# pmelchior/scarlet

Hardware: AMD Instinct MI355X
Metric: PGM iters/sec over batched blends; achieved HBM GB/s vs roofline (higher is better)
Workload: dtype f32; 1 GPU; configs[2]: 1024 independent 5-band 128x128 blends in total, 10 ExtendedSource components (41x41) each, ConvolutionRenderer FFT 160x160; iterations 0..1234 of a fit from the initial parameters; loop=blend, blends_total=1024, components_per_blend=10, sub_ranges_per_gpu=3

## Files before the change

include/scarlet_amd.h:

```cpp
#ifndef SCARLET_AMD_H
#define SCARLET_AMD_H

#include <stdint.h>

#ifdef __cplusplus
extern "C" {
#endif

typedef enum smi_status {
    SMI_OK = 0,
    SMI_ERR_INVALID = -1,
    SMI_ERR_HIP = -2,
    SMI_ERR_NO_DEVICE = -3,
    SMI_ERR_ARITHMETIC = -4
} smi_status;

const char *smi_last_error(void);
int smi_device_count(void);
const char *smi_version(void);


int smi_prox_weighted_monotonic_f32(float *flat_img, const float *weights,
                                    const int32_t *offsets, int32_t n_off,
                                    const int32_t *dist_idx, int32_t n_idx,
// ... 382 lines not shown
int smi_batch_set_iteration_base(smi_batch *b, const int32_t *base);
int smi_batch_get_progress(smi_batch *b, int32_t *state, int32_t *n_loss);
int smi_batch_set_pause_at(smi_batch *b, const int32_t *it);
int smi_batch_get_converged(smi_batch *b, int32_t *flag);
int smi_batch_set_round(smi_batch *b, const int32_t *state, const int32_t *base,
                        const int32_t *pause_at);
int smi_batch_get_round(smi_batch *b, int32_t *state, int32_t *n_loss, int32_t *converged);

int64_t smi_observation_uploads(void);

int smi_batch_conv_path_used(smi_batch *b, int32_t *path);

int smi_batch_set_frame_extents(smi_batch *b, const int32_t *h, const int32_t *w);

int smi_fft_shape_for(int32_t H, int32_t W, int32_t kernel_h, int32_t kernel_w, int32_t conv_path,
                      int32_t *Fy, int32_t *Fx);

typedef struct smi_resampler smi_resampler;
int smi_resampler_create(const float *A, const float *Pt, int32_t C, int32_t n_a, int32_t n_b,
                         int32_t Fy, int32_t Fx, smi_resampler **out);
int smi_resampler_render(smi_resampler *r, const float *model, float *out);
int smi_resampler_time(smi_resampler *r, int32_t n_rep, double *ms_per_render);
int smi_resampler_destroy(smi_resampler *r);
int smi_resampler_get_path(smi_resampler *r, int32_t *path);
int smi_resampler_set_path(smi_resampler *r, int32_t path);

int smi_gemm_plan(int32_t M, int32_t N, int32_t K, int32_t n_batch, int64_t scratch_elems,
                  int32_t plan[5]);
int smi_gemm_test(const float *A, int64_t strideA, const float *B, int64_t strideB, float *C,
                  int64_t strideC, int32_t n_batch, int32_t M, int32_t N, int32_t K,
                  int64_t scratch_elems, int32_t plan[5], int32_t *guard_ok);
int smi_resampler_adjoint(smi_resampler *r, const float *resid, float *gpad);

int smi_batch_attach_lowres(smi_batch *b, smi_resampler *r, const int32_t *channels,
                            const float *data, const float *weights, double log_norm);
int smi_batch_get_lowres_rendered(smi_batch *b, int32_t index, float *out);


int smi_starlet_transform_f32(const float *d_images, int32_t n, int32_t H, int32_t W,
                              int32_t scales, int32_t generation, double *d_coeffs,
                              double *d_work, void *stream);
int smi_starlet_transform_f64(const double *d_images, int32_t n, int32_t H, int32_t W,
                              int32_t scales, int32_t generation, double *d_coeffs,
                              double *d_work, void *stream);
int smi_starlet_reconstruction_f64(const double *d_coeffs, int32_t n, int32_t H, int32_t W,
                                   int32_t scales, int32_t generation, double *d_image,
                                   double *d_work, void *stream);
int smi_multiresolution_support_f64(const double *d_coeffs, int32_t n, int32_t planes,
                                    int32_t H, int32_t W, int64_t plane_stride,
                                    int64_t image_stride, const double *sigma0,
                                    const double *thresh0, double K, double epsilon,
                                    int32_t max_iter, int32_t *d_support, double *d_masked,
                                    int32_t *iterations, void *stream);
int smi_coadd_f32(const float *d_images, int32_t bands, int32_t H, int32_t W, float *d_out,
                  void *stream);
int smi_coadd_f64(const double *d_images, int32_t bands, int32_t H, int32_t W, double *d_out,
                  void *stream);

typedef struct smi_detect_task {
    int32_t bands, h, w, scales;
    int64_t image_off, coeff_off, work_off;
    double sigma0, thresh0;
} smi_detect_task;
int smi_detect_wavelets_scratch_bytes(int32_t n, int64_t *bytes);
int smi_detect_wavelets_f32(int32_t n, const smi_detect_task *tasks, const void *d_tasks, double K,
                            double epsilon, int32_t max_iter, int32_t generation,
// ... 71 lines not shown
```

scarlet_amd/_lib.py:

```python

import ctypes
import os

import numpy as np

_HERE = os.path.dirname(os.path.abspath(__file__))
LIB_PATH = os.environ.get("SCARLET_AMD_LIB") or os.path.join(_HERE, "libscarlet_amd.so")

PROX_MONOTONIC = 1
PROX_SYMMETRY = 2
PROX_POSITIVE = 4
PROX_CENTER_ON = 8
PROX_NORM_MAX = 16
PROX_NORM_SUM = 32
PROX_L1 = 64
PROX_L0 = 128
PROX_FIT_CENTER = 256
PROX_BG_THRESH = 512
PROX_L_RELATIVE = 1024
PROX_MONO_MASK = 2048
SCHEME_AMSGRAD, SCHEME_FISTA = 0, 1
COMPONENT_POINT_SOURCE = 1 << 16
COMPONENT_SHIFTING = 1 << 17
COMPONENT_FIXED_SED = 1 << 18
# ... 129 lines not shown
    "smi_get_valid_monotonic_pixels_f64": (
        ctypes.c_int,
        [ctypes.c_int32, ctypes.c_int32, c_f64p, ctypes.c_int32, ctypes.c_int32, c_u8p, c_u8p,
         ctypes.c_double, c_i32p, ctypes.c_double],
    ),
    "smi_linear_interpolate_invalid_pixels_f32": (
        ctypes.c_int,
        [c_i32p, c_i32p, ctypes.c_int32, c_u8p, c_f32p, ctypes.c_int32, ctypes.c_int32, c_u8p,
         ctypes.c_double, ctypes.c_int32, c_i32p],
    ),
    "smi_linear_interpolate_invalid_pixels_f64": (
        ctypes.c_int,
        [c_i32p, c_i32p, ctypes.c_int32, c_u8p, c_f64p, ctypes.c_int32, ctypes.c_int32, c_u8p,
         ctypes.c_double, ctypes.c_int32, c_i32p],
    ),
    "smi_resampler_create": (
        ctypes.c_int,
        [c_f32p, c_f32p, ctypes.c_int32, ctypes.c_int32, ctypes.c_int32, ctypes.c_int32,
         ctypes.c_int32, ctypes.POINTER(ctypes.c_void_p)],
    ),
    "smi_resampler_render": (ctypes.c_int, [ctypes.c_void_p, c_f32p, c_f32p]),
    "smi_resampler_time": (ctypes.c_int, [ctypes.c_void_p, ctypes.c_int32,
                                          ctypes.POINTER(ctypes.c_double)]),
    "smi_resampler_destroy": (ctypes.c_int, [ctypes.c_void_p]),
    "smi_resampler_get_path": (ctypes.c_int, [ctypes.c_void_p, ctypes.POINTER(ctypes.c_int32)]),
    "smi_resampler_set_path": (ctypes.c_int, [ctypes.c_void_p, ctypes.c_int32]),
    "smi_resampler_adjoint": (ctypes.c_int, [ctypes.c_void_p, c_f32p, c_f32p]),
    "smi_gemm_plan": (ctypes.c_int, [ctypes.c_int32] * 4 + [ctypes.c_int64, c_i32p]),
    "smi_gemm_test": (
        ctypes.c_int,
        [c_f32p, ctypes.c_int64, c_f32p, ctypes.c_int64, c_f32p, ctypes.c_int64]
        + [ctypes.c_int32] * 4 + [ctypes.c_int64, c_i32p, c_i32p],
    ),
    "smi_batch_attach_lowres": (
        ctypes.c_int, [ctypes.c_void_p, ctypes.c_void_p, c_i32p, c_f32p, c_f32p, ctypes.c_double]
    ),
    "smi_batch_get_lowres_rendered": (ctypes.c_int, [ctypes.c_void_p, ctypes.c_int32, c_f32p]),
    "smi_batch_create": (
        ctypes.c_int,
        [ctypes.POINTER(BatchDesc), ctypes.c_int, ctypes.POINTER(ctypes.c_void_p)],
    ),
    "smi_batch_destroy": (ctypes.c_int, [ctypes.c_void_p]),
    "smi_batch_add_sweep_plan": (
        ctypes.c_int,
        [ctypes.c_void_p, ctypes.c_int32, ctypes.c_int32, c_f64p, c_i32p, c_i32p,
         ctypes.c_int32],
    ),
    "smi_sweep_ring_plan": (
        ctypes.c_int,
        [ctypes.c_int32, ctypes.c_int32, c_f64p, c_i32p, c_i32p, ctypes.c_int32, c_i32p, c_f32p,
         ctypes.POINTER(ctypes.c_uint16), ctypes.c_int64],
    ),
    "smi_batch_set_observation": (ctypes.c_int, [ctypes.c_void_p, c_f32p, c_f32p]),
    "smi_batch_set_observation_device": (
        ctypes.c_int, [ctypes.c_void_p, ctypes.c_void_p, ctypes.c_void_p]
    ),
    "smi_batch_set_kernel": (ctypes.c_int, [ctypes.c_void_p, c_f32p]),
    "smi_batch_set_components": (ctypes.c_int, [ctypes.c_void_p, ctypes.POINTER(Components)]),
    "smi_batch_set_moments": (ctypes.c_int, [ctypes.c_void_p] + [c_f32p] * 6),
    "smi_batch_get_moments": (ctypes.c_int, [ctypes.c_void_p] + [c_f32p] * 6),
    "smi_batch_get_parameters": (ctypes.c_int, [ctypes.c_void_p, c_f32p, c_f32p]),
    "smi_batch_set_parameters": (ctypes.c_int, [ctypes.c_void_p, c_f32p, c_f32p]),
    "smi_batch_get_centers": (ctypes.c_int, [ctypes.c_void_p] + [c_f64p] * 5),
    "smi_batch_set_center_moments": (ctypes.c_int, [ctypes.c_void_p] + [c_f64p] * 3),
    "smi_batch_set_centers": (ctypes.c_int, [ctypes.c_void_p, c_f64p]),
    "smi_batch_get_model_morphology": (ctypes.c_int, [ctypes.c_void_p, c_f32p]),
# ... 235 lines not shown
```

scarlet_amd/csrc/batch.hip:

```cpp
#include <rocfft/rocfft.h>

#include <algorithm>
#include <cmath>
#include <cstdlib>
#include <atomic>
#include <cstring>
#include <limits>
#include <map>
#include <mutex>
#include <thread>
#include <tuple>
#include <utility>

#include "common.h"

namespace smi {

static thread_local std::string g_error;
static std::atomic<int> g_hw_queues{4};
static std::atomic<long long> g_observation_uploads{0};
static std::mutex g_plan_mutex;
void set_error(const std::string &msg) { g_error = msg; }

static int next_fast_len(int n) {
// ... 597 lines not shown
}

int smi_resampler_adjoint(smi_resampler *r, const float *resid, float *gpad) {
    SMI_REQUIRE(r && r->impl && resid && gpad, "null argument");
    return resampler_adjoint_host(r->impl, resid, gpad);
}

int smi_gemm_plan(int32_t M, int32_t N, int32_t K, int32_t n_batch, int64_t scratch_elems,
                  int32_t plan[5]) {
    SMI_REQUIRE(plan && scratch_elems >= 0, "bad argument");
    GemmPlan p;
    const int rc = gemm_plan(M, N, K, n_batch, (size_t)scratch_elems, &p);
    plan[0] = p.tm; plan[1] = p.tn; plan[2] = p.bk; plan[3] = p.kslice; plan[4] = p.n_slices;
    return rc;
}

int smi_gemm_test(const float *A, int64_t strideA, const float *B, int64_t strideB, float *C,
                  int64_t strideC, int32_t n_batch, int32_t M, int32_t N, int32_t K,
                  int64_t scratch_elems, int32_t plan[5], int32_t *guard_ok) {
    SMI_REQUIRE(A && B && C && plan && guard_ok && scratch_elems >= 0, "bad argument");
    int ndev = 0;
    if (hipGetDeviceCount(&ndev) != hipSuccess || ndev == 0) {
        set_error("no HIP device available");
        return SMI_ERR_NO_DEVICE;
    }
    GemmPlan p;
    *guard_ok = 0;
    const int rc = gemm_test(A, strideA, B, strideB, C, strideC, n_batch, M, N, K,
                             (size_t)scratch_elems, &p, guard_ok);
    plan[0] = p.tm; plan[1] = p.tn; plan[2] = p.bk; plan[3] = p.kslice; plan[4] = p.n_slices;
    return rc;
}

static constexpr int kMaxLowRes = 8;

int smi_batch_attach_lowres(smi_batch *b, smi_resampler *r, const int32_t *channels,
                            const float *data, const float *weights, double log_norm) {
    SMI_REQUIRE(b && r && channels && data && weights, "null argument");
    SMI_REQUIRE(b->d.n_blends == 1, "a low-resolution observation needs a batch of one blend");
    SMI_REQUIRE(!b->frame_hw, "a low-resolution observation does not support frame extents");
    SMI_REQUIRE(r->impl, "resampler already destroyed");
    SMI_REQUIRE((int)b->lowres.size() < kMaxLowRes, "too many low-resolution observations");
    SMI_HIP(hipSetDevice(b->device));
    SMI_HIP(hipStreamSynchronize(b->stream));
    if (!b->extra_terms) {
        SMI_HIP(dev_alloc(&b->extra_terms, kMaxLowRes));
        SMI_HIP(hipMemset(b->extra_terms, 0, kMaxLowRes * sizeof(double)));
    }
    LowRes *l = nullptr;
    int rc = lowres_create(r->impl, channels, data, weights, log_norm, b->d.H, b->d.W,
                           b->extra_terms + b->lowres.size(), &l);
    if (rc) {
        lowres_destroy(l);
        return rc;
    }
    b->lowres.push_back(l);
    refresh_view(b);
    return SMI_OK;
}

int smi_batch_get_lowres_rendered(smi_batch *b, int32_t index, float *out) {
    SMI_REQUIRE(b && out, "null argument");
    SMI_REQUIRE(index >= 0 && index < (int)b->lowres.size(), "no such low-resolution observation");
    return lowres_get_rendered(b->lowres[index], out, b->stream);
}

// ... 2320 lines not shown
```

scarlet_amd/csrc/common.h:

```cpp
#pragma once

#include <hip/hip_runtime.h>
#include <stdint.h>

#include <string>
#include <vector>

#include "../../include/scarlet_amd.h"

namespace smi {

void set_error(const std::string &msg);

#define SMI_HIP(expr)                                                              \
    do {                                                                           \
        hipError_t _e = (expr);                                                    \
        if (_e != hipSuccess) {                                                    \
            smi::set_error(std::string(#expr) + ": " + hipGetErrorString(_e));     \
            return SMI_ERR_HIP;                                                    \
        }                                                                          \
    } while (0)

#define SMI_REQUIRE(cond, msg)                                                     \
    do {                                                                           \
// ... 265 lines not shown
                            uint8_t *unchecked, uint8_t *orphans, double variance,
                            int32_t *bounds, double thresh);
template <typename T>
int mask_interpolate_host_buffers(const int32_t *row_idx, const int32_t *col_idx, int32_t n_idx,
                                  uint8_t *unchecked, T *model, int32_t rows, int32_t cols,
                                  uint8_t *orphans, double variance, int32_t recursive,
                                  int32_t *bounds);
struct Resampler;
int resampler_create(const float *A, const float *Pt, int C, int n_a, int n_b, int Fy, int Fx,
                     Resampler **out);
int resampler_render(Resampler *r, const float *model, float *out);
int resampler_time(Resampler *r, int n_rep, double *ms_per_render);
int resampler_get_path(const Resampler *r);
int resampler_set_path(Resampler *r, int path);
void resampler_destroy(Resampler *r);
int resampler_adjoint_host(Resampler *r, const float *resid, float *gpad);
struct GemmPlan {
    int32_t tm = 0, tn = 0, bk = 0, kslice = 0, n_slices = 0;
};
int gemm_plan(int M, int N, int K, int n_batch, size_t scratch_elems, GemmPlan *p);
int gemm_test(const float *A, int64_t strideA, const float *B, int64_t strideB, float *C,
              int64_t strideC, int n_batch, int M, int N, int K, size_t scratch_elems,
              GemmPlan *plan, int32_t *guard_ok);
struct LowRes;
int lowres_create(Resampler *r, const int32_t *channels, const float *data, const float *weights,
                  double log_norm, int H, int W, double *term_slot, LowRes **out);
void lowres_destroy(LowRes *l);
int lowres_evaluate(LowRes *l, const float *P, int Py, int Px, int backward, hipStream_t s);
void lowres_add_gradient(LowRes *l, float *Q, int Py, int Px, hipStream_t s);
int lowres_get_rendered(LowRes *l, float *out, hipStream_t s);
int launch_sweep_timing(const SweepPlanDev *d_plans, const SweepPlanDev &host_plan, int plan_id,
                        int mode, int n_rep, float one_minus_g, int waves, int groups,
                        long long *cycles, float *images, hipStream_t s);
void launch_resize_test(const BatchView &v, int32_t *margin, double *pull, hipStream_t s);
void launch_gather_states(const BatchView &v, const int32_t *sel, const int64_t *off, int32_t n_sel,
                          float *staging, hipStream_t s);
void launch_scatter_states(const BatchView &v, const int64_t *off, const float *staging,
                           hipStream_t s);
void launch_carry_states(const int32_t *keep, const int64_t *old_moff, const int64_t *new_moff,
                         int32_t n, float *const from[4], float *const to[4], hipStream_t s);
void launch_interleave_obs(const float *data, const float *weights, float4 *dw, int64_t planes,
                           int32_t H, int32_t W, hipStream_t s);
void launch_log_norm(const float *weights, double *log_norm, int32_t nb, int64_t n,
                     hipStream_t s);
void launch_wrap_kernel(const float *kern, float *out, int32_t n_img, int32_t ph,
                        int32_t pw, int32_t Fy, int32_t Fx, float scale, hipStream_t s);
void launch_crop(const float *P, float *out, int32_t n_img, int32_t H, int32_t W,
                 int32_t Fy, int32_t Fx, hipStream_t s);
void launch_count_active(const int32_t *state, int32_t nb, int32_t *out, hipStream_t s);

bool fused_conv_supported(int Fy, int Fx);
bool fused_conv_instantiated(int Fy, int Fx);
bool fused_conv_choose(int ny, int nx, int *Fy, int *Fx);
int launch_fused_conv(const BatchView &v, int Fy, int Fx, const float *model, const float2 *Kt,
                      int k_bands, int k_per_blend, float *out, int mode, long long *dbg,
                      hipStream_t s);
int launch_fused_conv_short(const BatchView &v, int Fy, int Fx, const float *model,
                            const float2 *Kt, int k_bands, int k_per_blend, float *out, int mode,
                            long long *dbg, hipStream_t s);
int launch_stamp_spectrum(const float *d_kern, double2 *d_tmp, float2 *Kt, int n_img, int ph,
                          int pw, int Fy, int Fx, double scale, hipStream_t s);
int launch_permute_kernel_spectrum(const float2 *Khat, float2 *Kt, int n_img, int Fy, int Fx,
                                   float scale, hipStream_t s);

template <typename T>
int sweep_host_buffers(T *flat_img, int32_t n_pix, const SweepPlanHost &plan, T min_gradient);
// ... 10 lines not shown
```

scarlet_amd/csrc/kernels.hip:

```cpp
#include <math.h>

#include <algorithm>
#include <type_traits>
#include <stdlib.h>

#include "common.h"
#include "rounded_math.h"

namespace smi {

namespace {

constexpr int kBandChunk = 8;
constexpr int kPixBlock = 256;

template <int CTRL>
__device__ __forceinline__ float dpp_f(float v) {
    return __int_as_float(__builtin_amdgcn_update_dpp(0, __float_as_int(v), CTRL, 0xf, 0xf, false));
}
__device__ __forceinline__ float wave_sum(float v) {
    v += dpp_f<0xB1>(v);
    v += dpp_f<0x4E>(v);
    v += dpp_f<0x141>(v);
    v += dpp_f<0x140>(v);
// ... 1273 lines not shown
    const RingGlobal<1> plan(stream, bytes, n_pad, lane);
    if (kLate && n_nat < n_pad)
        sweep_ring_loop<1, true, RingGlobal<1>>(us, plan, n_pad, n_nat, rmax, perm, centre,
                                                one_minus_g, lane);
    else
        sweep_ring_loop<1, false, RingGlobal<1>>(us, plan, n_pad, n_pad, rmax, perm, centre,
                                                 one_minus_g, lane);
}

#ifndef SMI_XP_TEAM
#define SMI_XP_TEAM 1
#endif
constexpr bool update_xp(int team) { return SMI_XP_TEAM && team > 64; }
constexpr int update_waves(int npl, int team) {
    return npl <= 16 ? 4 : npl <= 27 ? (update_xp(team) ? 4 : 3) : 2;
}
#ifndef SMI_WAVES
#define SMI_WAVES __attribute__((amdgpu_waves_per_eu(update_waves(NPL, T))))
#endif
template <int NPL, bool XP>
struct UpdState {
    CompCtx c;
    int k, flags, plan_id, bad, ctr, n_slots;
    float xs[XP ? 1 : NPL], rs[XP ? 1 : NPL], zs[NPL];
    float rpmax;
    bool fista_prox;
    float alpha, pmax, t_old;
    bool monotonic, fit_center;
    bool std_chain;
    const SweepSlotEntry *slots;
    const SweepPlanDev *ring;
    const SweepPlanDev *staged;
    const char *plan_lds;
    float one_minus_g, lthresh, cfloor, pfloor;
    const float *bg_level;
    float *us, *sed_new;
};

constexpr bool update_lean(int npl, int mode, int team) {
    return mode != 2 && !(team == 256 && npl == 16);
}
template <int T, bool LEAN>
__device__ __forceinline__ uint32_t slot_offset(int lane, uint32_t lane4, int j) {
    return LEAN ? lane4 + (uint32_t)(T * j) * 4u : (uint32_t)(lane + T * j) * 4u;
}
template <int NPL>
struct UpdFull {
    static constexpr int value = NPL == 7 ? 0 : NPL == 16 ? 7 : NPL == 27 ? 16 : NPL == 42 ? 27 : 42;
};

template <int NPL, int MODE, int T, bool EXT>
__device__ __forceinline__ void upd_step(const BatchView &v, const float *G, int it, float e2,
                                         int prox_max_iter, UpdState<NPL, update_xp(T)> &S) {
    constexpr bool LITE = MODE != 0;
    constexpr bool fista = MODE == 2;
    constexpr bool XP = update_xp(T);
    constexpr int kFull = UpdFull<NPL>::value;
    constexpr bool LEAN = update_lean(NPL, MODE, T);
    const CompCtx &c = S.c;
    it = v.local_it(c.b, it);
    const int lane = c.lane, k = S.k, N = c.N;
    const uint32_t lane4 = lane_byte_offset(lane);
    float *us = S.us;
    float xs_local[NPL], rs_local[NPL];
    auto &xs = [&]() -> float(&)[NPL] {
        if constexpr (XP) return xs_local;
        else return S.xs;
    }();
    auto &rs = [&]() -> float(&)[NPL] {
        if constexpr (XP) return rs_local;
        else return S.rs;
    }();
    float(&zs)[NPL] = S.zs;
    const int flags = S.flags = v.c_flags[k];
    const int plan_id = S.plan_id = v.c_plan[k];
    const uint32_t nbytes = (uint32_t)N * 4u;

    {
        const rsrc_t r_morph = make_rsrc(c.morph, nbytes);
#pragma unroll
        for (int j = 0; j < NPL; ++j) zs[j] = buf_load(r_morph, slot_offset<T, LEAN>(lane, lane4, j));
    }
    float g_sed = 0.f;
    if (c.pre) {
        const rsrc_t r_g = make_rsrc(v.g_morph_buf + c.moff, nbytes);
#pragma unroll
        for (int j = 0; j < NPL; ++j) xs[j] = buf_load(r_g, slot_offset<T, LEAN>(lane, lane4, j));
        g_sed = lane < c.C ? v.g_sed_buf[(int64_t)k * c.C + lane] : 0.f;
    } else {
        uint32_t *goff = reinterpret_cast<uint32_t *>(us);
        const float inv_w = 1.0f / (float)c.w;
        const int Hb = EXT ? v.frame_h(c.b) : v.H, Wb = EXT ? v.frame_w(c.b) : v.W;
#pragma unroll
        for (int j = 0; j < NPL; ++j) {
            const int i = lane + T * j;
            const int y = (int)(((float)i + 0.5f) * inv_w);
            const int x = i - y * c.w;
            const int fy = y + c.oy, fx = x + c.ox;
            const bool ok = (j < kFull || i < N) && (unsigned)fy < (unsigned)Hb &&
                            (unsigned)fx < (unsigned)Wb;
            goff[i] = ok ? (uint32_t)(fy * v.Fx + fx) * 4u : kOutOfRange;
            xs[j] = 0.f;
        }
        const int64_t plane = (int64_t)v.Fy * v.Fx;
        for (int cb = 0; cb < c.C; ++cb) {
            const rsrc_t r_g = make_rsrc(G + ((int64_t)c.b * c.C + cb) * plane, (uint32_t)plane * 4u);
            float g[NPL];
#pragma unroll
            for (int j = 0; j < NPL; ++j) g[j] = buf_load(r_g, goff[lane + T * j]);
            const float s = c.sed[cb];
            float acc = 0.f;
#pragma unroll
            for (int j = 0; j < NPL; ++j) {
                xs[j] = fmaf(s, g[j], xs[j]);
                acc = fmaf(g[j], zs[j], acc);
            }
            const float t = Team<T>::sum(acc);
            if (lane == cb) g_sed = t;
        }
    }
    if (flags & SMI_COMPONENT_FIXED_MORPH) {
#pragma unroll
        for (int j = 0; j < NPL; ++j) xs[j] = 0.f;
    }
    if (flags & SMI_COMPONENT_FIXED_SED) g_sed = 0.f;

    float msum = 0.f, msum2 = 0.f;
#pragma unroll
    for (int j = 0; j < NPL; ++j) {
        msum += zs[j];
        msum2 = fmaf(zs[j], zs[j], msum2);
    }
    float ssum2 = 1.f;
    S.t_old = 1.f;
    if (fista) {
        msum2 = Team<T>::sum(msum2);
        const float so = lane < c.C ? c.sed[lane] : 0.f;
        ssum2 = Team<T>::sum(so * so);
        S.t_old = (float)v.fista_t[2 * (int64_t)k + 1];
    }
    S.bad = 0;
    if (T == 64 || threadIdx.x < 64)
        S.bad = update_spectrum(v, c, g_sed, it, e2, prox_max_iter, msum2, S.sed_new);
    const float alpha = fmaxf(v.c_morph_step[k], v.c_morph_rel[k] * (Team<T>::sum(msum) / (float)N));
    float pmax = 0.f;
    const rsrc_t r_m = make_rsrc(v.m_morph + c.moff, nbytes);
    const rsrc_t r_x = make_rsrc(v.xp_tmp + c.moff, nbytes);
    const rsrc_t r_p = make_rsrc(v.xp_tmp + v.n_morph_total + c.moff, nbytes);
    S.fista_prox = fista;
    if (fista) {
        const float step = v.c_fista_step[k] / ssum2;
        if constexpr (XP) {
#pragma unroll
            for (int j = 0; j < NPL; ++j) zs[j] = buf_load(r_m, slot_offset<T, LEAN>(lane, lane4, j));
#pragma unroll
            for (int j = 0; j < NPL; ++j) zs[j] = zs[j] - step * xs[j];
        } else {
#pragma unroll
            for (int j = 0; j < NPL; ++j) rs[j] = buf_load(r_m, slot_offset<T, LEAN>(lane, lane4, j));
#pragma unroll
            for (int j = 0; j < NPL; ++j) {
                xs[j] = rs[j] - step * xs[j];
                rs[j] = 0.f;
                zs[j] = xs[j];
            }
        }
        pmax = 1.f;
    } else {
        const rsrc_t r_v = make_rsrc(v.v_morph + c.moff, nbytes);
        const rsrc_t r_vh = make_rsrc(v.vh_morph + c.moff, nbytes);
        constexpr int CH = NPL <= 6 ? NPL : 6;
        const float b1 = v.b1, b2 = v.b2, eps = v.eps;
        float cm[CH], cv[CH], cvh[CH];
#pragma unroll
        for (int u = 0; u < CH; ++u) {
            const uint32_t off = slot_offset<T, LEAN>(lane, lane4, u);
            cm[u] = buf_load(r_m, off);
            cv[u] = buf_load(r_v, off);
            cvh[u] = buf_load(r_vh, off);
        }
#pragma unroll
        for (int j0 = 0; j0 < NPL; j0 += CH) {
            float nm[CH], nv[CH], nvh[CH];
#pragma unroll
            for (int u = 0; u < CH; ++u) {
                nm[u] = nv[u] = nvh[u] = 0.f;
                if (j0 + CH + u < NPL) {
                    const uint32_t off = slot_offset<T, LEAN>(lane, lane4, (j0 + CH + u));
                    nm[u] = buf_load(r_m, off);
                    nv[u] = buf_load(r_v, off);
                    nvh[u] = buf_load(r_vh, off);
                }
            }
#pragma unroll
            for (int u = 0; u < CH; ++u) {
                const int j = j0 + u;
                if (j < NPL) {
                    const uint32_t off = slot_offset<T, LEAN>(lane, lane4, j);
                    const float g = xs[j];
                    const float m = (1.f - b1) * g + b1 * cm[u];
                    const float vv = (1.f - b2) * g * g + b2 * cv[u];
                    const float vh = it == 0 ? vv : fmaxf(cvh[u], vv);
                    buf_store(r_m, off, m);
                    buf_store(r_v, off, vv);
                    buf_store(r_vh, off, vh);
                    const float psi = sqrtf(fmaxf(vh, eps));
                    float upd = alpha * m / psi;
                    if (it == 0) upd /= 10.f;
                    xs[j] = zs[j] - upd;
                    zs[j] = xs[j];
                    const bool in_box = j < kFull || lane + T * j < N;
                    if constexpr (XP) {
                        const float rj = in_box ? psi : 0.f;
                        buf_store(r_x, off, xs[j]);
                        buf_store(r_p, off, rj);
                        pmax = fmaxf(pmax, rj);
                    } else {
                        rs[j] = in_box ? psi : 0.f;
                        pmax = fmaxf(pmax, rs[j]);
                    }
                }
            }
#pragma unroll
            for (int u = 0; u < CH; ++u) {
                cm[u] = nm[u];
                cv[u] = nv[u];
                cvh[u] = nvh[u];
            }
            __builtin_amdgcn_sched_barrier(0);
        }
        pmax = Team<T>::max(pmax);
    }
    const float rpmax = 1.f / pmax;
    S.rpmax = rpmax;
    if constexpr (!XP) {
#pragma unroll
        for (int j = 0; j < NPL; ++j) rs[j] = rs[j] * rpmax;
    }
    S.alpha = alpha;
    S.pmax = pmax;

    S.monotonic = (flags & SMI_PROX_MONOTONIC) && plan_id >= 0;
    S.fit_center = LITE && S.monotonic && (flags & SMI_PROX_FIT_CENTER);
    S.slots = nullptr;
    S.ring = nullptr;
    S.n_slots = 0;
    if (S.monotonic && !S.fit_center) {
        S.slots = v.plans[plan_id].slots;
        S.n_slots = v.plans[plan_id].n_slots;
        S.ring = v.plans[plan_id].ring ? &v.plans[plan_id] : nullptr;
    }
    constexpr int kChainLinks = SMI_PROX_SYMMETRY | SMI_PROX_POSITIVE | SMI_PROX_CENTER_ON |
// ... 169 lines not shown
    const uint32_t lane4 = lane_byte_offset(lane);
    const uint32_t nbytes = (uint32_t)c.N * 4u;
    float omega = 0.f;
    if (fista) {
        const float t_old = S.t_old;
        const float tn = 0.5f * (1.f + sqrtf(1.f + 4.f * t_old * t_old));
        omega = 1.f + (t_old - 1.f) / tn;
        if (lane == 0) v.fista_t[2 * (int64_t)S.k + 1] = (double)tn;
    }
    const rsrc_t r_out = make_rsrc(c.morph_out, nbytes);
    if (fista) {
        const rsrc_t r_m = make_rsrc(v.m_morph + c.moff, nbytes);
        float xo[NPL];
#pragma unroll
        for (int j = 0; j < NPL; ++j) xo[j] = buf_load(r_out, slot_offset<T, LEAN>(lane, lane4, j));
#pragma unroll
        for (int j = 0; j < NPL; ++j)
            buf_store(r_m, slot_offset<T, LEAN>(lane, lane4, j), xo[j] + omega * (S.zs[j] - xo[j]));
    }
    int bad = S.bad;
#pragma unroll
    for (int j = 0; j < NPL; ++j) {
        buf_store(r_out, slot_offset<T, LEAN>(lane, lane4, j), S.zs[j]);
        bad |= !isfinite(S.zs[j]);
    }
    if (Team<T>::any(bad) && lane == 0) atomicExch(&v.state[c.b], v.fail_code);
}

template <int NPL, int MODE, int T = 64, bool kGlobalRing = false, bool EXT = false>
__device__ __forceinline__ void update_component(const BatchView &v, const float *G, int it,
                                                 float e_rel, int prox_max_iter, int k,
                                                 float *us, float *sed_new,
                                                 const SweepPlanDev *staged = nullptr,
                                                 const char *plan_lds = nullptr, int tid = -1) {
    constexpr bool fista = MODE == 2;
    UpdState<NPL, update_xp(T)> S;
    S.k = k;
    S.staged = staged;
    S.plan_lds = plan_lds;
    if (tid < 0) tid = (int)threadIdx.x;
    S.c = comp_ctx(v, k, T == 64 ? (tid & 63) : tid);
    if (v.state[S.c.b] >= 2) return;
    S.us = us;
    S.sed_new = sed_new;
    const float e2 = e_rel * e_rel;
    if (fista) prox_max_iter = 1;
    upd_step<NPL, MODE, T, EXT>(v, G, it, e2, prox_max_iter, S);
    team_fence<T>();
    for (int tau = 0; tau < prox_max_iter; ++tau) {
        upd_prox_begin<NPL, MODE, T>(v, S);
        team_fence<T>();
        upd_prox_plan(v, S);
        if (S.monotonic) {
            if (T == 64 || threadIdx.x < 64) {
                if (S.ring && S.ring == S.staged)
                    sweep_ring<1, (NPL > 27)>(S.us, *S.ring, S.plan_lds, S.one_minus_g, S.c.lane);
                else if (kGlobalRing && T == 64 && S.ring &&
                         __builtin_amdgcn_readfirstlane(S.ring->ring_planes) == 1)
                    sweep_ring_global<(NPL > 27)>(S.us, *S.ring, S.one_minus_g, S.c.lane);
                else
                    sweep_slots(S.us, S.slots, S.n_slots, S.one_minus_g, S.c.lane);
            }
            if (T > 64) __syncthreads();
        }
        if (upd_prox_end<NPL, MODE, T>(v, e2, S)) break;
    }
    upd_store<NPL, MODE, T>(v, S);
}

__device__ __forceinline__ int xcd_contiguous(int b, int n) {
    const int q = n >> 3, r = n & 7, x = b & 7;
    return x * q + min(x, r) + (b >> 3);
}

constexpr int update_pack_max(int npl, int team) {
    return team != 64 ? 1 : 4 * update_waves(npl, team);
}
template <int NPL, int MODE, int T, bool EXT>
__global__ __launch_bounds__(T * update_pack_max(NPL, T)) SMI_WAVES void update_kernel_reg(
    BatchView v, const float *G, int it, float e_rel, int prox_max_iter, int n_items,
    int n_finalize, int min_iter, int check, int stage_plan, int persistent) {
    constexpr int kPack = update_pack_max(NPL, T);
    __shared__ float sed_new[kPack][64];
    __shared__ int next_item;
    const int wave = T == 64 ? __builtin_amdgcn_readfirstlane((int)(threadIdx.x >> 6)) : 0;
    const int pack = T == 64 ? (int)(blockDim.x >> 6) : 1;
    const int n_blocks = (int)gridDim.x - n_finalize;
    if ((int)blockIdx.x >= n_blocks) {
        if (threadIdx.x < 64)
            finalize_blend(v, (int)blockIdx.x - n_blocks + v.blend0, it, e_rel, min_iter, check);
        return;
    }
    float *us = lds_dyn + wave * (T * NPL + 4) + 4;
    const SweepPlanDev *staged = nullptr;
    const char *plan_lds = nullptr;
    if (T == 64 && (stage_plan >= 0 || persistent)) {
        if (threadIdx.x == 0) next_item = 0;
        if (stage_plan >= 0) {
            staged = &v.plans[stage_plan];
            u32x4 *dst = reinterpret_cast<u32x4 *>(lds_dyn + pack * (T * NPL + 4));
            const u32x4 *src = static_cast<const u32x4 *>(staged->ring);
            const uint32_t n16 = staged->ring_bytes >> 4;
            for (uint32_t i = threadIdx.x; i < n16; i += blockDim.x) dst[i] = src[i];
            plan_lds = reinterpret_cast<const char *>(dst);
        }
        __syncthreads();
    }
    const bool loop = T == 64 && persistent;
    const int q = n_items / n_blocks, r = n_items % n_blocks;
    const int b = loop ? xcd_contiguous((int)blockIdx.x, n_blocks) : (int)blockIdx.x;
    const int lo = loop ? b * q + (b < r ? b : r) : 0;
    const int hi = loop ? lo + q + (b < r) : n_items;
    const int lane = (int)(threadIdx.x & 63);
    for (;;) {
        int k = xcd_contiguous(blockIdx.x, n_blocks) * pack + wave;
        if (loop) {
            if (lane == 0) k = atomicAdd(&next_item, 1);
            k = __builtin_amdgcn_readfirstlane(k);
        }
        if (lo + k >= hi) break;
        int tid = (int)threadIdx.x;
        asm volatile("" : "+v"(tid));
        update_component<NPL, MODE, T, false, EXT>(v, G, it, e_rel, prox_max_iter, v.work[lo + k + v.work0],
                                       us, sed_new[wave], staged, plan_lds, tid);
        if (!loop) break;
    }
}

template <int MODE, int WAVES, bool EXT>
__global__ __launch_bounds__(64) __attribute__((amdgpu_waves_per_eu(WAVES))) void update_kernel_mixed(
    BatchView v, const float *G, int it, float e_rel, int prox_max_iter, int n_finalize,
    int min_iter, int check) {
    __shared__ float sed_new[64];
    if ((int)blockIdx.x >= v.n_comp) {
        finalize_blend(v, (int)blockIdx.x - v.n_comp + v.blend0, it, e_rel, min_iter, check);
        return;
    }
    const int k = v.comp0 + blockIdx.x;
    if (v.c_flags[k] & SMI_COMPONENT_POINT_SOURCE) return;
    const int n = v.c_h[k] * v.c_w[k];
    float *us = lds_dyn + 4;
    if (n <= 64 * kUpdateNpl[0])
        update_component<kUpdateNpl[0], MODE, 64, true, EXT>(v, G, it, e_rel, prox_max_iter, k, us, sed_new);
    else if (n <= 64 * kUpdateNpl[1])
        update_component<kUpdateNpl[1], MODE, 64, true, EXT>(v, G, it, e_rel, prox_max_iter, k, us, sed_new);
    else if (n <= 64 * kUpdateNpl[2])
        update_component<kUpdateNpl[2], MODE, 64, true, EXT>(v, G, it, e_rel, prox_max_iter, k, us, sed_new);
    else if (n <= 64 * kUpdateNpl[3])
        update_component<kUpdateNpl[3], MODE, 64, true, EXT>(v, G, it, e_rel, prox_max_iter, k, us, sed_new);
    else
        update_component<kUpdateNpl[4], MODE, 64, true, EXT>(v, G, it, e_rel, prox_max_iter, k, us, sed_new);
}

__global__ void sweep_timing_kernel(const SweepPlanDev *plans, int plan_id, int mode, int n_rep,
                                    float one_minus_g, long long *cycles, float *images) {
    const SweepPlanDev &pl = plans[plan_id];
    const int lane = threadIdx.x & 63;
    const int wave = __builtin_amdgcn_readfirstlane((int)(threadIdx.x >> 6));
    const int n = pl.h * pl.w, stride = ((n + 3) & ~3) + 4;
    float *us = lds_dyn + wave * stride + 4;
    const int gw = blockIdx.x * (blockDim.x >> 6) + wave;
    us[-4 + (lane & 3)] = 0.f;
    char *plan_lds = reinterpret_cast<char *>(lds_dyn + (blockDim.x >> 6) * stride);
    if (mode == 2) {
        const uint32_t *src = static_cast<const uint32_t *>(pl.ring);
        for (uint32_t i = threadIdx.x; i < pl.ring_bytes / 4; i += blockDim.x)
            reinterpret_cast<uint32_t *>(plan_lds)[i] = src[i];
        __syncthreads();
    }
    long long total = 0;
    for (int rep = 0; rep < n_rep; ++rep) {
        for (int i = lane; i < n; i += 64) {
            uint32_t hsh = (uint32_t)(i * 2654435761u) ^ (uint32_t)(gw * 40503u + rep * 977u);
            hsh ^= hsh >> 13;
            hsh *= 0x5bd1e995u;
            hsh ^= hsh >> 15;
            us[i] = (float)(hsh & 0xffff) * (1.f / 65536.f);
        }
        wave_lds_fence();
        const long long t0 = __builtin_readcyclecounter();
        if (mode == 3)
            sweep_ring_global<true>(us, pl, one_minus_g, lane);
        else if (mode == 2)
            sweep_ring<2, true>(us, pl, plan_lds, one_minus_g, lane);
// ... 424 lines not shown
    constexpr int kPack = update_pack_max(NPL, T);
    int pack = n_items <= kUpdatePackLimit ? kPack : 1;
    if (forced > 0) pack = std::min(forced, kPack);
    int stage = -1, persistent = 0;
    int n_blocks = (n_items + pack - 1) / pack;
    size_t lds = (size_t)pack * (T * NPL + 4) * sizeof(float);
    if (T == 64 && may_stage && v.stage_plan[cls] >= 0) {
        const size_t per_wave = (size_t)(T * NPL + 4) * sizeof(float);
        const size_t fixed = (size_t)kPack * 64 * sizeof(float) + 64 + v.stage_bytes[cls];
        const int fit = fixed < 160 * 1024 ? (int)((160 * 1024 - fixed) / per_wave) : 0;
        if (fit >= 4) {
            stage = v.stage_plan[cls];
            pack = std::min(forced > 0 ? pack : kPack, fit);
            lds = (size_t)pack * per_wave + v.stage_bytes[cls];
            n_blocks = (n_items + pack - 1) / pack;
            const int resident = cu_count() * std::max(1, (int)((160 * 1024) / (lds + kPack * 256 + 64)));
            static const bool may_persist = [] {
                const char *e = getenv("SMI_PERSIST");
                return !e || atoi(e) != 0;
            }();
            static const int forced_blocks = [] {
                const char *e = getenv("SMI_PERSIST_BLOCKS");
                return e ? atoi(e) : 0;
            }();
            if (forced_blocks > 0 && n_blocks > forced_blocks) {
                n_blocks = forced_blocks;
                persistent = 1;
            } else if (n_blocks > resident && may_persist) {
                n_blocks = resident;
                persistent = 1;
            }
        }
    }
    const dim3 grid(n_blocks + n_fin), block(T * pack);
#define SMI_LAUNCH_EXT(MODE, EXT)                                                               \
    {                                                                                           \
        static size_t configured[kMaxDevices] = {};                                             \
        auto kern = update_kernel_reg<NPL, MODE, T, EXT>;                                       \
        if (lds > 48 * 1024)                                                                    \
            if (int rc = ensure_dynamic_lds(reinterpret_cast<const void *>(kern), lds, configured)) \
                return rc;                                                                      \
        hipLaunchKernelGGL(kern, grid, block, lds, s, vi, G, it, e_rel, prox_max_iter, n_items, \
                           n_fin, fin.min_iter, fin.check, stage, persistent);                         \
    }
#define SMI_LAUNCH(MODE)                                                                        \
    if (v.frame_hw) SMI_LAUNCH_EXT(MODE, true)                                                  \
    else SMI_LAUNCH_EXT(MODE, false)
    if (v.scheme == SMI_SCHEME_FISTA) SMI_LAUNCH(2)
    else if (v.lite) SMI_LAUNCH(1)
    else SMI_LAUNCH(0)
#undef SMI_LAUNCH
#undef SMI_LAUNCH_EXT
    return SMI_OK;
}

int launch_update_finalize(const BatchView &v, const float *G, int32_t it, float e_rel,
                           int32_t min_iter, int32_t check, int32_t prox_max_iter,
                           hipStream_t s) {
    static const int mode = [] {
        const char *e = getenv("SMI_FOLD_FINALIZE");
        return e ? atoi(e) : 2;
    }();
    if (mode == 0 || (mode == 2 && v.n_comp > kUpdatePackLimit)) {
        launch_finalize(v, it, e_rel, min_iter, check, s);
        return launch_update(v, G, it, e_rel, prox_max_iter, nullptr, nullptr, 0, s);
    }
    pending_finalize.on = true;
    pending_finalize.min_iter = min_iter;
    pending_finalize.check = check;
    const int rc = launch_update(v, G, it, e_rel, prox_max_iter, nullptr, nullptr, 0, s);
    const bool left = pending_finalize.on;
    pending_finalize.on = false;
    if (rc) return rc;
    if (left) launch_finalize(v, it, e_rel, min_iter, check, s);
    return SMI_OK;
}
// ... 128 lines not shown
}

int launch_point_sources(const BatchView &v_in, const float *G, int32_t it, float e_rel,
                         int32_t prox_max_iter, float *g_sed_out, double *g_center_out,
                         int32_t mode, hipStream_t s) {
    if (v_in.n_point == 0 || v_in.n_comp == 0) return SMI_OK;
    BatchView v = v_in;
    v.fail_code = 3 + std::max(it, 0);
    const size_t lds = (size_t)(((v.max_box_pixels + 3) & ~3) + 4) * sizeof(float);
    SMI_REQUIRE(lds <= 64 * 1024, "component box too large for the point-source kernel");
    hipLaunchKernelGGL(point_source_kernel, dim3(v.n_comp), dim3(64), lds, s, v, G, it, e_rel,
                       prox_max_iter, g_sed_out, g_center_out, mode);
    return SMI_OK;
}

int launch_sweep_timing(const SweepPlanDev *d_plans, const SweepPlanDev &host_plan, int plan_id,
                        int mode, int n_rep, float one_minus_g, int waves, int groups,
                        long long *cycles, float *images, hipStream_t s) {
    const int n = host_plan.h * host_plan.w;
    const size_t lds = (size_t)waves * (((n + 3) & ~3) + 4) * sizeof(float) +
                       (mode == 2 ? host_plan.ring_bytes : 0);
    SMI_REQUIRE(lds <= 160 * 1024 && waves >= 1 && waves <= 16, "images do not fit the LDS");
    SMI_REQUIRE(mode == 0 || mode == 2 || (mode == 3 && host_plan.ring_planes == 1),
                "mode: 0 slot plan, 2 ring schedule, 3 ring schedule with the stream in L2 (one plane)");
    SMI_REQUIRE(mode == 0 ? host_plan.slots != nullptr : host_plan.ring != nullptr, "plan has no such schedule");
    static size_t configured[kMaxDevices] = {};
    if (int rc = ensure_dynamic_lds(reinterpret_cast<const void *>(sweep_timing_kernel), lds, configured))
        return rc;
    hipLaunchKernelGGL(sweep_timing_kernel, dim3(groups), dim3(64 * waves), lds, s, d_plans, plan_id,
                       mode, n_rep, one_minus_g, cycles, images);
    return SMI_OK;
}

void launch_resize_test(const BatchView &v, int32_t *margin, double *pull, hipStream_t s) {
    if (v.n_comp)
        hipLaunchKernelGGL(resize_test_kernel, dim3(v.n_comp), dim3(64), 0, s, v, margin, pull);
}

void launch_gather_states(const BatchView &v, const int32_t *sel, const int64_t *off, int32_t n_sel,
                          float *staging, hipStream_t s) {
    if (n_sel)
        hipLaunchKernelGGL(gather_states_kernel, dim3(n_sel), dim3(256), 0, s, v, sel, off, staging);
}

void launch_scatter_states(const BatchView &v, const int64_t *off, const float *staging,
                           hipStream_t s) {
    if (v.n_comp)
        hipLaunchKernelGGL(scatter_states_kernel, dim3(v.n_comp), dim3(256), 0, s, v, off, staging);
}

void launch_carry_states(const int32_t *keep, const int64_t *old_moff, const int64_t *new_moff,
                         int32_t n, float *const from[4], float *const to[4], hipStream_t s) {
    PixelArrays a, b;
    for (int i = 0; i < 4; ++i) {
        a.p[i] = from[i];
        b.p[i] = to[i];
    }
    if (n)
        hipLaunchKernelGGL(carry_states_kernel, dim3(n), dim3(256), 0, s, keep, old_moff, new_moff, a, b);
}

void launch_interleave_obs(const float *data, const float *weights, float4 *dw, int64_t planes,
                           int32_t H, int32_t W, hipStream_t s) {
    const int blocks = std::max(1, std::min(((H + 1) / 2 * W + 255) / 256, 64));
    for (int64_t p0 = 0; p0 < planes; p0 += 65535) {
        const int np = (int)std::min<int64_t>(planes - p0, 65535);
// ... 192 lines not shown
```

scarlet_amd/csrc/rounded_math.h:

```cpp
#pragma once

#include <hip/hip_runtime.h>

namespace smi {

__device__ __forceinline__ float mul_rn(float a, float b) { return __fmul_rn(a, b); }
__device__ __forceinline__ double mul_rn(double a, double b) { return __dmul_rn(a, b); }
__device__ __forceinline__ float add_rn(float a, float b) { return __fadd_rn(a, b); }
__device__ __forceinline__ double add_rn(double a, double b) { return __dadd_rn(a, b); }
__device__ __forceinline__ float div_rn(float a, float b) { return __fdiv_rn(a, b); }
__device__ __forceinline__ double div_rn(double a, double b) { return __ddiv_rn(a, b); }

}
```

Measured before the change: 1.398 million blend-iterations/s.

## Precompute gather offset table in LDS and use faster correctly-rounded sqrt in AMSGrad step

For 64-lane update teams with a staged sweep plan, the kernel now builds a per-block LDS table of gradient gather offsets for the staged box shape. Components whose box matches and sits fully inside the frame read offsets from that table through a base-shifted buffer resource, instead of recomputing the y/x division and bounds checks per pixel. The AMSGrad step is also restructured into groups of three. When eps is large enough to rule out denormals, it uses a hardware sqrt with a one-ulp fma correction in place of the library sqrtf, and it hoists the it==0 test into a wave-uniform flag. This adds LDS use, which is only granted when occupancy does not drop, plus a new exported test entry point for checking that the sqrt is correctly rounded.

```diff
diff --git a/include/scarlet_amd.h b/include/scarlet_amd.h
--- a/include/scarlet_amd.h
+++ b/include/scarlet_amd.h
@@ -438,6 +438,8 @@
                   int64_t scratch_elems, int32_t plan[5], int32_t *guard_ok);
 int smi_resampler_adjoint(smi_resampler *r, const float *resid, float *gpad);
 
+int smi_sqrt_rn_normal_test(const float *x, float *y, int64_t n);
+
 int smi_batch_attach_lowres(smi_batch *b, smi_resampler *r, const int32_t *channels,
                             const float *data, const float *weights, double log_norm);
 int smi_batch_get_lowres_rendered(smi_batch *b, int32_t index, float *out);
diff --git a/scarlet_amd/_lib.py b/scarlet_amd/_lib.py
--- a/scarlet_amd/_lib.py
+++ b/scarlet_amd/_lib.py
@@ -185,6 +185,7 @@
         [c_f32p, ctypes.c_int64, c_f32p, ctypes.c_int64, c_f32p, ctypes.c_int64]
         + [ctypes.c_int32] * 4 + [ctypes.c_int64, c_i32p, c_i32p],
     ),
+    "smi_sqrt_rn_normal_test": (ctypes.c_int, [c_f32p, c_f32p, ctypes.c_int64]),
     "smi_batch_attach_lowres": (
         ctypes.c_int, [ctypes.c_void_p, ctypes.c_void_p, c_i32p, c_f32p, c_f32p, ctypes.c_double]
     ),
diff --git a/scarlet_amd/csrc/batch.hip b/scarlet_amd/csrc/batch.hip
--- a/scarlet_amd/csrc/batch.hip
+++ b/scarlet_amd/csrc/batch.hip
@@ -653,6 +653,12 @@
     return rc;
 }
 
+int smi_sqrt_rn_normal_test(const float *x, float *y, int64_t n) {
+    SMI_REQUIRE(x && y, "null argument");
+    if (int rc = have_device()) return rc;
+    return sqrt_rn_normal_test(x, y, n);
+}
+
 static constexpr int kMaxLowRes = 8;
 
 int smi_batch_attach_lowres(smi_batch *b, smi_resampler *r, const int32_t *channels,
diff --git a/scarlet_amd/csrc/common.h b/scarlet_amd/csrc/common.h
--- a/scarlet_amd/csrc/common.h
+++ b/scarlet_amd/csrc/common.h
@@ -321,6 +321,7 @@
 int launch_sweep_timing(const SweepPlanDev *d_plans, const SweepPlanDev &host_plan, int plan_id,
                         int mode, int n_rep, float one_minus_g, int waves, int groups,
                         long long *cycles, float *images, hipStream_t s);
+int sqrt_rn_normal_test(const float *x, float *y, int64_t n);
 void launch_resize_test(const BatchView &v, int32_t *margin, double *pull, hipStream_t s);
 void launch_gather_states(const BatchView &v, const int32_t *sel, const int64_t *off, int32_t n_sel,
                           float *staging, hipStream_t s);
diff --git a/scarlet_amd/csrc/kernels.hip b/scarlet_amd/csrc/kernels.hip
--- a/scarlet_amd/csrc/kernels.hip
+++ b/scarlet_amd/csrc/kernels.hip
@@ -1329,6 +1329,7 @@
     const SweepPlanDev *ring;
     const SweepPlanDev *staged;
     const char *plan_lds;
+    const uint32_t *gtab;
     float one_minus_g, lthresh, cfloor, pfloor;
     const float *bg_level;
     float *us, *sed_new;
@@ -1337,6 +1338,12 @@
 constexpr bool update_lean(int npl, int mode, int team) {
     return mode != 2 && !(team == 256 && npl == 16);
 }
+constexpr bool update_step_lean(int npl, int mode, int team) {
+    return mode != 2 && team == 64 && !(npl == 7 && mode == 1);
+}
+constexpr bool update_gather_table(int npl, int mode, int team) {
+    return team == 64 && npl < 59;
+}
 template <int T, bool LEAN>
 __device__ __forceinline__ uint32_t slot_offset(int lane, uint32_t lane4, int j) {
     return LEAN ? lane4 + (uint32_t)(T * j) * 4u : (uint32_t)(lane + T * j) * 4u;
@@ -1346,7 +1353,7 @@
     static constexpr int value = NPL == 7 ? 0 : NPL == 16 ? 7 : NPL == 27 ? 16 : NPL == 42 ? 27 : 42;
 };
 
-template <int NPL, int MODE, int T, bool EXT>
+template <int NPL, int MODE, int T, bool EXT, bool MIXED>
 __device__ __forceinline__ void upd_step(const BatchView &v, const float *G, int it, float e2,
                                          int prox_max_iter, UpdState<NPL, update_xp(T)> &S) {
     constexpr bool LITE = MODE != 0;
@@ -1354,6 +1361,8 @@
     constexpr bool XP = update_xp(T);
     constexpr int kFull = UpdFull<NPL>::value;
     constexpr bool LEAN = update_lean(NPL, MODE, T);
+    constexpr bool STEP_LEAN = !MIXED && update_step_lean(NPL, MODE, T);
+    constexpr bool GTAB = !MIXED && update_gather_table(NPL, MODE, T);
     const CompCtx &c = S.c;
     it = v.local_it(c.b, it);
     const int lane = c.lane, k = S.k, N = c.N;
@@ -1386,25 +1395,41 @@
         g_sed = lane < c.C ? v.g_sed_buf[(int64_t)k * c.C + lane] : 0.f;
     } else {
         uint32_t *goff = reinterpret_cast<uint32_t *>(us);
-        const float inv_w = 1.0f / (float)c.w;
         const int Hb = EXT ? v.frame_h(c.b) : v.H, Wb = EXT ? v.frame_w(c.b) : v.W;
-#pragma unroll
-        for (int j = 0; j < NPL; ++j) {
-            const int i = lane + T * j;
-            const int y = (int)(((float)i + 0.5f) * inv_w);
-            const int x = i - y * c.w;
-            const int fy = y + c.oy, fx = x + c.ox;
-            const bool ok = (j < kFull || i < N) && (unsigned)fy < (unsigned)Hb &&
-                            (unsigned)fx < (unsigned)Wb;
-            goff[i] = ok ? (uint32_t)(fy * v.Fx + fx) * 4u : kOutOfRange;
-            xs[j] = 0.f;
+        const uint32_t *offs = goff;
+        int64_t first_px = 0;
+        bool table = false;
+        if constexpr (GTAB) {
+            table = S.gtab && c.h == S.staged->h && c.w == S.staged->w && c.oy >= 0 && c.ox >= 0 &&
+                    c.oy + c.h <= Hb && c.ox + c.w <= Wb;
+            table = __builtin_amdgcn_readfirstlane((int)table) != 0;
+        }
+        if (table) {
+            offs = S.gtab;
+            first_px = (int64_t)c.oy * v.Fx + c.ox;
+#pragma unroll
+            for (int j = 0; j < NPL; ++j) xs[j] = 0.f;
+        } else {
+            const float inv_w = 1.0f / (float)c.w;
+#pragma unroll
+            for (int j = 0; j < NPL; ++j) {
+                const int i = lane + T * j;
+                const int y = (int)(((float)i + 0.5f) * inv_w);
+                const int x = i - y * c.w;
+                const int fy = y + c.oy, fx = x + c.ox;
+                const bool ok = (j < kFull || i < N) && (unsigned)fy < (unsigned)Hb &&
+                                (unsigned)fx < (unsigned)Wb;
+                goff[i] = ok ? (uint32_t)(fy * v.Fx + fx) * 4u : kOutOfRange;
+                xs[j] = 0.f;
+            }
         }
         const int64_t plane = (int64_t)v.Fy * v.Fx;
         for (int cb = 0; cb < c.C; ++cb) {
-            const rsrc_t r_g = make_rsrc(G + ((int64_t)c.b * c.C + cb) * plane, (uint32_t)plane * 4u);
+            const rsrc_t r_g = make_rsrc(G + ((int64_t)c.b * c.C + cb) * plane + first_px,
+                                         (uint32_t)(plane - first_px) * 4u);
             float g[NPL];
 #pragma unroll
-            for (int j = 0; j < NPL; ++j) g[j] = buf_load(r_g, goff[lane + T * j]);
+            for (int j = 0; j < NPL; ++j) g[j] = buf_load(r_g, offs[lane + T * j]);
             const float s = c.sed[cb];
             float acc = 0.f;
 #pragma unroll
@@ -1468,6 +1493,9 @@
         const rsrc_t r_vh = make_rsrc(v.vh_morph + c.moff, nbytes);
         constexpr int CH = NPL <= 6 ? NPL : 6;
         const float b1 = v.b1, b2 = v.b2, eps = v.eps;
+        const bool first = __builtin_amdgcn_readfirstlane((int)(it == 0)) != 0;
+        const bool normal_sqrt =
+            __builtin_amdgcn_readfirstlane((int)(eps >= kSqrtNormalMin)) != 0;
         float cm[CH], cv[CH], cvh[CH];
 #pragma unroll
         for (int u = 0; u < CH; ++u) {
@@ -1489,32 +1517,98 @@
                     nvh[u] = buf_load(r_vh, off);
                 }
             }
-#pragma unroll
-            for (int u = 0; u < CH; ++u) {
-                const int j = j0 + u;
-                if (j < NPL) {
-                    const uint32_t off = slot_offset<T, LEAN>(lane, lane4, j);
-                    const float g = xs[j];
-                    const float m = (1.f - b1) * g + b1 * cm[u];
-                    const float vv = (1.f - b2) * g * g + b2 * cv[u];
-                    const float vh = it == 0 ? vv : fmaxf(cvh[u], vv);
-                    buf_store(r_m, off, m);
-                    buf_store(r_v, off, vv);
-                    buf_store(r_vh, off, vh);
-                    const float psi = sqrtf(fmaxf(vh, eps));
-                    float upd = alpha * m / psi;
-                    if (it == 0) upd /= 10.f;
-                    xs[j] = zs[j] - upd;
-                    zs[j] = xs[j];
-                    const bool in_box = j < kFull || lane + T * j < N;
-                    if constexpr (XP) {
-                        const float rj = in_box ? psi : 0.f;
-                        buf_store(r_x, off, xs[j]);
-                        buf_store(r_p, off, rj);
-                        pmax = fmaxf(pmax, rj);
+            if constexpr (STEP_LEAN) {
+                constexpr int SUB = 3;
+                static_assert(CH % SUB == 0, "whole sub-groups");
+#pragma unroll
+                for (int u0 = 0; u0 < CH; u0 += SUB) {
+                    float w[SUB];
+#pragma unroll
+                    for (int q = 0; q < SUB; ++q) {
+                        const int u = u0 + q, j = j0 + u;
+                        if (j < NPL) {
+                            const uint32_t off = slot_offset<T, LEAN>(lane, lane4, j);
+                            const float g = xs[j];
+                            const float m = (1.f - b1) * g + b1 * cm[u];
+                            const float vv = (1.f - b2) * g * g + b2 * cv[u];
+                            const float vh = first ? vv : fmaxf(cvh[u], vv);
+                            buf_store(r_m, off, m);
+                            buf_store(r_v, off, vv);
+                            buf_store(r_vh, off, vh);
+                            w[q] = fmaxf(vh, eps);
+                            xs[j] = alpha * m;
+                        }
+                    }
+                    if (normal_sqrt) {
+#pragma unroll
+                        for (int q = 0; q < SUB; ++q)
+                            if (j0 + u0 + q < NPL) w[q] = sqrt_rn_normal(w[q]);
                     } else {
-                        rs[j] = in_box ? psi : 0.f;
-                        pmax = fmaxf(pmax, rs[j]);
+#pragma unroll
+                        for (int q = 0; q < SUB; ++q)
+                            if (j0 + u0 + q < NPL) {
+                                w[q] = sqrtf(w[q]);
+                                asm volatile("" : "+v"(w[q]));
+                            }
+                    }
+#pragma unroll
+                    for (int q = 0; q < SUB; ++q)
+                        if (j0 + u0 + q < NPL) xs[j0 + u0 + q] = xs[j0 + u0 + q] / w[q];
+                    if (first) {
+#pragma unroll
+                        for (int q = 0; q < SUB; ++q)
+                            if (j0 + u0 + q < NPL) {
+                                xs[j0 + u0 + q] = xs[j0 + u0 + q] / 10.f;
+                                asm volatile("" : "+v"(xs[j0 + u0 + q]));
+                            }
+                    }
+#pragma unroll
+                    for (int q = 0; q < SUB; ++q) {
+                        const int j = j0 + u0 + q;
+                        if (j < NPL) {
+                            xs[j] = zs[j] - xs[j];
+                            zs[j] = xs[j];
+                            const bool in_box = j < kFull || lane + T * j < N;
+                            const float rj = in_box ? w[q] : 0.f;
+                            if constexpr (XP) {
+                                const uint32_t off = slot_offset<T, LEAN>(lane, lane4, j);
+                                buf_store(r_x, off, xs[j]);
+                                buf_store(r_p, off, rj);
+                            } else {
+                                rs[j] = rj;
+                            }
+                            pmax = fmaxf(pmax, rj);
+                        }
+                    }
+                }
+            } else {
+#pragma unroll
+                for (int u = 0; u < CH; ++u) {
+                    const int j = j0 + u;
+                    if (j < NPL) {
+                        const uint32_t off = slot_offset<T, LEAN>(lane, lane4, j);
+                        const float g = xs[j];
+                        const float m = (1.f - b1) * g + b1 * cm[u];
+                        const float vv = (1.f - b2) * g * g + b2 * cv[u];
+                        const float vh = it == 0 ? vv : fmaxf(cvh[u], vv);
+                        buf_store(r_m, off, m);
+                        buf_store(r_v, off, vv);
+                        buf_store(r_vh, off, vh);
+                        const float psi = sqrtf(fmaxf(vh, eps));
+                        float upd = alpha * m / psi;
+                        if (it == 0) upd /= 10.f;
+                        xs[j] = zs[j] - upd;
+                        zs[j] = xs[j];
+                        const bool in_box = j < kFull || lane + T * j < N;
+                        if constexpr (XP) {
+                            const float rj = in_box ? psi : 0.f;
+                            buf_store(r_x, off, xs[j]);
+                            buf_store(r_p, off, rj);
+                            pmax = fmaxf(pmax, rj);
+                        } else {
+                            rs[j] = in_box ? psi : 0.f;
+                            pmax = fmaxf(pmax, rs[j]);
+                        }
                     }
                 }
             }
@@ -1750,12 +1844,14 @@
                                                  float e_rel, int prox_max_iter, int k,
                                                  float *us, float *sed_new,
                                                  const SweepPlanDev *staged = nullptr,
-                                                 const char *plan_lds = nullptr, int tid = -1) {
+                                                 const char *plan_lds = nullptr, int tid = -1,
+                                                 const uint32_t *gtab = nullptr) {
     constexpr bool fista = MODE == 2;
     UpdState<NPL, update_xp(T)> S;
     S.k = k;
     S.staged = staged;
     S.plan_lds = plan_lds;
+    S.gtab = gtab;
     if (tid < 0) tid = (int)threadIdx.x;
     S.c = comp_ctx(v, k, T == 64 ? (tid & 63) : tid);
     if (v.state[S.c.b] >= 2) return;
@@ -1763,7 +1859,7 @@
     S.sed_new = sed_new;
     const float e2 = e_rel * e_rel;
     if (fista) prox_max_iter = 1;
-    upd_step<NPL, MODE, T, EXT>(v, G, it, e2, prox_max_iter, S);
+    upd_step<NPL, MODE, T, EXT, kGlobalRing>(v, G, it, e2, prox_max_iter, S);
     team_fence<T>();
     for (int tau = 0; tau < prox_max_iter; ++tau) {
         upd_prox_begin<NPL, MODE, T>(v, S);
@@ -1797,7 +1893,7 @@
 template <int NPL, int MODE, int T, bool EXT>
 __global__ __launch_bounds__(T * update_pack_max(NPL, T)) SMI_WAVES void update_kernel_reg(
     BatchView v, const float *G, int it, float e_rel, int prox_max_iter, int n_items,
-    int n_finalize, int min_iter, int check, int stage_plan, int persistent) {
+    int n_finalize, int min_iter, int check, int stage_plan, int persistent, int gather_off) {
     constexpr int kPack = update_pack_max(NPL, T);
     __shared__ float sed_new[kPack][64];
     __shared__ int next_item;
@@ -1812,6 +1908,7 @@
     float *us = lds_dyn + wave * (T * NPL + 4) + 4;
     const SweepPlanDev *staged = nullptr;
     const char *plan_lds = nullptr;
+    const uint32_t *gtab = nullptr;
     if (T == 64 && (stage_plan >= 0 || persistent)) {
         if (threadIdx.x == 0) next_item = 0;
         if (stage_plan >= 0) {
@@ -1821,6 +1918,18 @@
             const uint32_t n16 = staged->ring_bytes >> 4;
             for (uint32_t i = threadIdx.x; i < n16; i += blockDim.x) dst[i] = src[i];
             plan_lds = reinterpret_cast<const char *>(dst);
+            if constexpr (update_gather_table(NPL, MODE, T)) {
+                if (gather_off >= 0) {
+                    uint32_t *tab = reinterpret_cast<uint32_t *>(lds_dyn) + (gather_off >> 2);
+                    const int w = staged->w, n = staged->h * w;
+                    const float inv_w = 1.0f / (float)w;
+                    for (int i = threadIdx.x; i < T * NPL; i += blockDim.x) {
+                        const int y = (int)(((float)i + 0.5f) * inv_w);
+                        tab[i] = i < n ? (uint32_t)(y * v.Fx + (i - y * w)) * 4u : kOutOfRange;
+                    }
+                    gtab = tab;
+                }
+            }
         }
         __syncthreads();
     }
@@ -1840,7 +1949,7 @@
         int tid = (int)threadIdx.x;
         asm volatile("" : "+v"(tid));
         update_component<NPL, MODE, T, false, EXT>(v, G, it, e_rel, prox_max_iter, v.work[lo + k + v.work0],
-                                       us, sed_new[wave], staged, plan_lds, tid);
+                                       us, sed_new[wave], staged, plan_lds, tid, gtab);
         if (!loop) break;
     }
 }
@@ -1868,6 +1977,11 @@
         update_component<kUpdateNpl[3], MODE, 64, true, EXT>(v, G, it, e_rel, prox_max_iter, k, us, sed_new);
     else
         update_component<kUpdateNpl[4], MODE, 64, true, EXT>(v, G, it, e_rel, prox_max_iter, k, us, sed_new);
+}
+
+__global__ __launch_bounds__(256) void sqrt_rn_normal_test_kernel(float *x, int64_t n) {
+    const int64_t i = (int64_t)blockIdx.x * 256 + threadIdx.x;
+    if (i < n) x[i] = sqrt_rn_normal(x[i]);
 }
 
 __global__ void sweep_timing_kernel(const SweepPlanDev *plans, int plan_id, int mode, int n_rep,
@@ -2358,16 +2472,32 @@
             }
         }
     }
+    int gather_off = -1;
+    size_t lds_table = lds;
+    if (stage >= 0) {
+        const size_t fixed = (size_t)kPack * 256 + 64;
+        const size_t off = (size_t)pack * (T * NPL + 4) * sizeof(float) +
+                           (((size_t)v.stage_bytes[cls] + 15) & ~(size_t)15);
+        const size_t with = off + (size_t)T * NPL * sizeof(uint32_t);
+        if (with + fixed <= 160 * 1024 &&
+            (160 * 1024) / (with + fixed) == (160 * 1024) / (lds + fixed)) {
+            gather_off = (int)off;
+            lds_table = with;
+        }
+    }
     const dim3 grid(n_blocks + n_fin), block(T * pack);
 #define SMI_LAUNCH_EXT(MODE, EXT)                                                               \
     {                                                                                           \
         static size_t configured[kMaxDevices] = {};                                             \
         auto kern = update_kernel_reg<NPL, MODE, T, EXT>;                                       \
-        if (lds > 48 * 1024)                                                                    \
-            if (int rc = ensure_dynamic_lds(reinterpret_cast<const void *>(kern), lds, configured)) \
+        const bool tab = update_gather_table(NPL, MODE, T) && gather_off >= 0;                  \
+        const size_t lds_k = tab ? lds_table : lds;                                             \
+        if (lds_k > 48 * 1024)                                                                  \
+            if (int rc = ensure_dynamic_lds(reinterpret_cast<const void *>(kern), lds_k, configured)) \
                 return rc;                                                                      \
-        hipLaunchKernelGGL(kern, grid, block, lds, s, vi, G, it, e_rel, prox_max_iter, n_items, \
-                           n_fin, fin.min_iter, fin.check, stage, persistent);                         \
+        hipLaunchKernelGGL(kern, grid, block, lds_k, s, vi, G, it, e_rel, prox_max_iter, n_items, \
+                           n_fin, fin.min_iter, fin.check, stage, persistent,                   \
+                           tab ? gather_off : -1);                                              \
     }
 #define SMI_LAUNCH(MODE)                                                                        \
     if (v.frame_hw) SMI_LAUNCH_EXT(MODE, true)                                                  \
@@ -2562,6 +2692,27 @@
     return SMI_OK;
 }
 
+int sqrt_rn_normal_test(const float *x, float *y, int64_t n) {
+    SMI_REQUIRE(n >= 0 && n < (int64_t)1 << 30, "sqrt_rn_normal_test: bad length");
+    if (n == 0) return SMI_OK;
+    float *d = nullptr;
+    SMI_HIP(hipMalloc((void **)&d, (size_t)n * sizeof(float)));
+    hipError_t e = hipMemcpy(d, x, (size_t)n * sizeof(float), hipMemcpyHostToDevice);
+    if (e == hipSuccess) {
+        hipLaunchKernelGGL(sqrt_rn_normal_test_kernel, dim3((unsigned)((n + 255) / 256)), dim3(256),
+                           0, nullptr, d, n);
+        e = hipGetLastError();
+    }
+    if (e == hipSuccess) e = hipDeviceSynchronize();
+    if (e == hipSuccess) e = hipMemcpy(y, d, (size_t)n * sizeof(float), hipMemcpyDeviceToHost);
+    (void)hipFree(d);
+    if (e != hipSuccess) {
+        set_error(std::string("sqrt_rn_normal_test: ") + hipGetErrorString(e));
+        return SMI_ERR_HIP;
+    }
+    return SMI_OK;
+}
+
 void launch_resize_test(const BatchView &v, int32_t *margin, double *pull, hipStream_t s) {
     if (v.n_comp)
         hipLaunchKernelGGL(resize_test_kernel, dim3(v.n_comp), dim3(64), 0, s, v, margin, pull);
diff --git a/scarlet_amd/csrc/rounded_math.h b/scarlet_amd/csrc/rounded_math.h
--- a/scarlet_amd/csrc/rounded_math.h
+++ b/scarlet_amd/csrc/rounded_math.h
@@ -11,4 +11,15 @@
 __device__ __forceinline__ float div_rn(float a, float b) { return __fdiv_rn(a, b); }
 __device__ __forceinline__ double div_rn(double a, double b) { return __ddiv_rn(a, b); }
 
+constexpr float kSqrtNormalMin = 0x1p-96f;
+__device__ __forceinline__ float sqrt_rn_normal(float x) {
+    const float s = __builtin_amdgcn_sqrtf(x);
+    const float dn = __uint_as_float(__float_as_uint(s) - 1u);
+    const float up = __uint_as_float(__float_as_uint(s) + 1u);
+    const float r_dn = fmaf(-dn, s, x), r_up = fmaf(-up, s, x);
+    float r = r_dn <= 0.f ? dn : s;
+    r = r_up > 0.f ? up : r;
+    return r;
 }
+
+}
```

After: 1.413 million blend-iterations/s (median of 6 runs). 1.0% higher.
